# JiehongLin/SAM-6D

Measured on AMD Instinct MI355X. Metric: RGB-D frames/sec (SAM-6D per-frame hot path: SAM ViT-H encoder + ISM scoring + PEM), higher is better.
Workload: dtype bf16 (SAM ViT-H: 87 % of the step) + f16 (PEM ViT-B feature extractor) + f32 (ISM scoring, PEM point transformer and pose solvers); 1 GPU; LM-O single object: 32 frames/step/GPU, 640x480 RGB-D -> 1024^2 SAM input, P=128 proposals x 42 templates (scored in groups of 8 frames), 1 instance/frame, 2048 pts (PEM batch 32); sam_frames_per_launch_group=16, pem_vit_dtype=fp16 (set by bench.py; the library default is fp32)

## Files before the change

### sam6d_amd/csrc/s6d_attn_win16.h

```cpp
#pragma once
#include "s6d_attn_common.h"

namespace S6D_ATTN_NS {

#ifndef S6D_WIN16_STREAM
#define S6D_WIN16_STREAM 1
#endif
#ifndef S6D_WIN16_KSWZ
#define S6D_WIN16_KSWZ 1
#endif

template <int HD>
struct RelFrags {
  union { uint4 u; bf16x8 v; } rh[2][Cfg<HD>::KS], rw[2][Cfg<HD>::KS];
  __device__ __forceinline__ void load(const AttnParams &p, int lane) {
    using C = Cfg<HD>;
    const int g = lane >> 4, c = lane & 15;
#pragma unroll
    for (int jt = 0; jt < 2; ++jt)
#pragma unroll
      for (int ks = 0; ks < C::KS; ++ks) {
        rh[jt][ks].u = *reinterpret_cast<const uint4 *>(p.rel_h + (size_t)(jt * 16 + c) * C::HDP + ks * 32 + g * 8);
        rw[jt][ks].u = *reinterpret_cast<const uint4 *>(p.rel_w + (size_t)(jt * 16 + c) * C::HDP + ks * 32 + g * 8);
      }
  }
};

constexpr int W16_LT = 36;

template <int HD, int NR, int SRC>
__device__ __forceinline__ void win16_tables(const RelFrags<HD> &rf, int S, int qy0, int rstride,
                                             const bf16x8 (*qf)[Cfg<HD>::KS], float *tab, float (*twr)[4],
                                             float (*thv)[16], int lane) {
  using C = Cfg<HD>;
  const int g = lane >> 4, c = lane & 15;
#pragma unroll
  for (int n = 0; n < NR; ++n) {
    const int qy = min(qy0 + n * rstride, S - 1);
    f32x4 ah[2], aw[2];
#pragma unroll
    for (int jt = 0; jt < 2; ++jt) {
      ah[jt] = f32x4{0.f, 0.f, 0.f, 0.f};
      aw[jt] = f32x4{0.f, 0.f, 0.f, 0.f};
#pragma unroll
      for (int ks = 0; ks < C::KS; ++ks) {
        aw[jt] = S6D_ATTN_MFMA16(rf.rw[jt][ks].v, qf[n][ks], aw[jt]);
        ah[jt] = S6D_ATTN_MFMA16(rf.rh[jt][ks].v, qf[n][ks], ah[jt]);
      }
    }
#pragma unroll
    for (int jt = 0; jt < 2; ++jt)
      *reinterpret_cast<float4 *>(tab + c * W16_LT + jt * 16 + g * 4) =
          make_float4(aw[jt][0] * kLog2e, aw[jt][1] * kLog2e, aw[jt][2] * kLog2e, aw[jt][3] * kLog2e);
    S6D_WAVE_RENDEZVOUS();
#pragma unroll
    for (int r = 0; r < 4; ++r) {
      const int kx = g * 4 + r;
      const float v = tab[c * W16_LT + min(max(c - kx + S - 1, 0), 31)];
      twr[n][r] = (kx < S && c < S) ? v : -1e30f;
    }
    S6D_WAVE_RENDEZVOUS();
#pragma unroll
    for (int jt = 0; jt < 2; ++jt)
      *reinterpret_cast<float4 *>(tab + c * W16_LT + jt * 16 + g * 4) =
          make_float4(ah[jt][0] * kLog2e, ah[jt][1] * kLog2e, ah[jt][2] * kLog2e, ah[jt][3] * kLog2e);
    S6D_WAVE_RENDEZVOUS();
#pragma unroll
    for (int ky = 0; ky < SRC; ++ky) {
      const float v = tab[c * W16_LT + min(max(qy - ky + S - 1, 0), 31)];
      thv[n][ky] = ky < S ? v : -1e30f;
    }
    S6D_WAVE_RENDEZVOUS();
  }
}

struct Win16NoMid {
  __device__ __forceinline__ void operator()() const {}
};
template <int HD, int NS, int SRC, bool EXACT, int KROWT = Cfg<HD>::KROW, bool KSWZ = false, class MID = Win16NoMid>
__device__ __forceinline__ void win16_pass(const AttnParams &p, const u16 *Kl, const u16 *Vl, int S, int SR, int b,
                                           int wy, int wx, int head, int qy0, int rstride,
                                           const bf16x8 (&qf)[NS][Cfg<HD>::KS], const float (*twr)[4],
                                           const float (*thv)[16], int lane, MID mid = MID()) {
  using C = Cfg<HD>;
  const int g = lane >> 4, c = lane & 15;
  const int Cc = p.nh * HD;
  float sp[NS][SRC][4], m[NS];
#pragma unroll
  for (int n = 0; n < NS; ++n) m[n] = -1e29f;
  f32x4 cb[NS];
  {
    const float inv = 1.0f / p.scale_log2;
#pragma unroll
    for (int n = 0; n < NS; ++n)
#pragma unroll
      for (int r = 0; r < 4; ++r) cb[n][r] = twr[n][r] * inv;
  }
  bf16x8 kf[2][C::KS];
  const int gk = KSWZ ? (g ^ kswz(c)) : g;
  auto kload = [&](int ky, bf16x8 (&dst)[C::KS]) {
    const int kyc = EXACT ? ky : min(ky, SR - 1);
#pragma unroll
    for (int ks = 0; ks < C::KS; ++ks) {
      dst[ks] = *reinterpret_cast<const bf16x8 *>(Kl + (kyc * 16 + c) * KROWT + ks * 32 + gk * 8);
      if (KROWT < C::HDP && ks * 32 + 32 > HD && ks * 32 + g * 8 >= HD) {
        union { bf16x8 v; uint4 u; } z;
        z.u = make_uint4(0, 0, 0, 0);
        dst[ks] = z.v;
      }
    }
  };
  kload(0, kf[0]);
#pragma unroll
  for (int ky = 0; ky < SRC; ++ky) {
    if (ky + 1 < SRC) kload(ky + 1, kf[(ky + 1) & 1]);
    f32x4 acc[NS];
#pragma unroll
    for (int n = 0; n < NS; ++n) acc[n] = cb[n];
#pragma unroll
    for (int ks = 0; ks < C::KS; ++ks)
#pragma unroll
      for (int n = 0; n < NS; ++n)
        acc[n] = S6D_ATTN_MFMA16(kf[ky & 1][ks], qf[n][ks], acc[n]);
#pragma unroll
    for (int n = 0; n < NS; ++n) {
#pragma unroll
      for (int r = 0; r < 4; ++r) sp[n][ky][r] = acc[n][r];
      const float mk = __builtin_fmaf(fmaxf(fmaxf(acc[n][0], acc[n][1]), fmaxf(acc[n][2], acc[n][3])), p.scale_log2, thv[n][ky]);
      m[n] = fmaxf(m[n], mk);
    }
  }
#pragma unroll
  for (int n = 0; n < NS; ++n) {
    m[n] = fmaxf(m[n], __shfl_xor(m[n], 16));
    m[n] = fmaxf(m[n], __shfl_xor(m[n], 32));
  }
  f32x4 oacc[NS][C::DT], lacc[NS];
#pragma unroll
  for (int n = 0; n < NS; ++n) {
    lacc[n] = f32x4{0.f, 0.f, 0.f, 0.f};
#pragma unroll
    for (int dt = 0; dt < C::DT; ++dt) oacc[n][dt] = f32x4{0.f, 0.f, 0.f, 0.f};
  }
  union { bf16x8 v; u16 hh[8]; } ones;
#pragma unroll
  for (int i = 0; i < 8; ++i) ones.hh[i] = S6D_ATTN_ONE;
#pragma unroll
  for (int u = 0; u < SRC; u += 2) {
    if (u == ((SRC / 2 + 1) & ~1)) {
      __builtin_amdgcn_sched_barrier(0);
      mid();
      __builtin_amdgcn_sched_barrier(0);
    }
    if (EXACT || u < SR) {
      union { bf16x8 v; s16x4 q[2]; } va[C::DT];
      const u16 *vrow = Vl + (u * 16 + g * 4 + (c >> 2)) * C::VROW + (c & 3) * 4;
#pragma unroll
      for (int dt = 0; dt < C::DT; ++dt) {
        va[dt].q[0] = __builtin_amdgcn_ds_read_tr16_b64_v4i16((S6D_LDS(s16x4) *)(vrow + dt * 16));
        va[dt].q[1] = __builtin_amdgcn_ds_read_tr16_b64_v4i16((S6D_LDS(s16x4) *)(vrow + 16 * C::VROW + dt * 16));
      }
      union { bf16x8 v; u16 hh[8]; } pb[NS];
#pragma unroll
      for (int n = 0; n < NS; ++n)
#pragma unroll
        for (int h = 0; h < 2; ++h) {
          const float nb = thv[n][u + h] - m[n];
          for (int r = 0; r < 4; ++r) pb[n].hh[h * 4 + r] = f2bf(fast_exp2(__builtin_fmaf(sp[n][u + h][r], p.scale_log2, nb)));
        }
#pragma unroll
      for (int n = 0; n < NS; ++n) lacc[n] = S6D_ATTN_MFMA16(ones.v, pb[n].v, lacc[n]);
#pragma unroll
      for (int dt = 0; dt < C::DT; ++dt)
#pragma unroll
        for (int n = 0; n < NS; ++n)
          oacc[n][dt] = S6D_ATTN_MFMA16(va[dt].v, pb[n].v, oacc[n][dt]);
    }
  }
#pragma unroll
  for (int n = 0; n < NS; ++n) {
    const int qy = qy0 + n * rstride;
    const int y = wy * p.ws + qy, x = wx * p.ws + c;
    if ((qy < S) && c < S && (y < p.H) && (x < p.W)) {
      const float inv = 1.0f / lacc[n][0];
      u16 *dst = p.out + ((size_t)(b * p.H + y) * p.W + x) * (size_t)Cc + head * HD;
#pragma unroll
      for (int dt = 0; dt < C::DT; ++dt) {
        union { uint2 u2; u16 hh[4]; } o;
#pragma unroll
        for (int r = 0; r < 4; ++r) o.hh[r] = f2bf(oacc[n][dt][r] * inv);
        *reinterpret_cast<uint2 *>(dst + dt * 16 + g * 4) = o.u2;
      }
    }
  }
}

template <int HD, int SRC, int KROWT, bool KSWZ, class NEXTQ, class THISQ>
__device__ __forceinline__ void win16_pass_stream(const AttnParams &p, const u16 *Kl, const u16 *Vl, int S, int b, int wy, int wx,
                                                  int head, int qy0, int rstride, const bf16x8 (&qf)[2][Cfg<HD>::KS],
                                                  const float (*twr)[4], const float (*thv)[16], int lane, NEXTQ next_q, THISQ this_q) {
  using C = Cfg<HD>;
  constexpr int NS = 2;
  static_assert(SRC % 2 == 0 && SRC >= 4, "whole 32-key steps");
  const int g = lane >> 4, c = lane & 15;
  const int Cc = p.nh * HD;
  const int gk = KSWZ ? (g ^ kswz(c)) : g;
  f32x4 cb[NS];
  {
    const float inv = 1.0f / p.scale_log2;
#pragma unroll
    for (int n = 0; n < NS; ++n)
#pragma unroll
      for (int r = 0; r < 4; ++r) cb[n][r] = twr[n][r] * inv;
  }
  bf16x8 kf[2][C::KS];
  auto kload = [&](int ky, bf16x8 (&dst)[C::KS]) __attribute__((always_inline)) {
#pragma unroll
    for (int ks = 0; ks < C::KS; ++ks) {
      dst[ks] = *reinterpret_cast<const bf16x8 *>(Kl + (ky * 16 + c) * KROWT + ks * 32 + gk * 8);
      if (KROWT < C::HDP && ks * 32 + 32 > HD && ks * 32 + g * 8 >= HD) {
        union { bf16x8 v; uint4 u; } z;
        z.u = make_uint4(0, 0, 0, 0);
        dst[ks] = z.v;
      }
    }
  };
  auto scores = [&](const bf16x8 (&k)[C::KS], f32x4 (&acc)[NS]) __attribute__((always_inline)) {
#pragma unroll
    for (int n = 0; n < NS; ++n) acc[n] = cb[n];
#pragma unroll
    for (int ks = 0; ks < C::KS; ++ks)
#pragma unroll
      for (int n = 0; n < NS; ++n) acc[n] = S6D_ATTN_MFMA16(k[ks], qf[n][ks], acc[n]);
  };
  f32x4 s0[NS], s1[NS];
  kload(0, kf[0]);
  kload(1, kf[1]);
  scores(kf[0], s0);
  scores(kf[1], s1);
  float m[NS];
#pragma unroll
  for (int n = 0; n < NS; ++n) {
    const float m0 = __builtin_fmaf(fmaxf(fmaxf(s0[n][0], s0[n][1]), fmaxf(s0[n][2], s0[n][3])), p.scale_log2, thv[n][0]);
    const float m1 = __builtin_fmaf(fmaxf(fmaxf(s1[n][0], s1[n][1]), fmaxf(s1[n][2], s1[n][3])), p.scale_log2, thv[n][1]);
    float v = fmaxf(fmaxf(m0, m1), -1e29f);
    v = fmaxf(v, __shfl_xor(v, 16));
    v = fmaxf(v, __shfl_xor(v, 32));
    m[n] = v;
  }
  union { bf16x8 v; u16 hh[8]; } ones;
#pragma unroll
  for (int i = 0; i < 8; ++i) ones.hh[i] = S6D_ATTN_ONE;
  f32x4 oacc[NS][C::DT], lacc[NS];
  int round = 0;
  for (;;) {
#pragma unroll
    for (int n = 0; n < NS; ++n) {
      lacc[n] = f32x4{0.f, 0.f, 0.f, 0.f};
#pragma unroll
      for (int dt = 0; dt < C::DT; ++dt) oacc[n][dt] = f32x4{0.f, 0.f, 0.f, 0.f};
    }
#pragma unroll
    for (int u = 0; u < SRC; u += 2) {
      if (u > 0 || round > 0) {
        kload(u, kf[0]);
        kload(u + 1, kf[1]);
        scores(kf[0], s0);
        scores(kf[1], s1);
      }
      if (u == SRC - 2 && round == 0) {
        __builtin_amdgcn_sched_barrier(0);
        next_q();
        __builtin_amdgcn_sched_barrier(0);
      }
      union { bf16x8 v; s16x4 q[2]; } va[C::DT];
      const u16 *vrow = Vl + (u * 16 + g * 4 + (c >> 2)) * C::VROW + (c & 3) * 4;
#pragma unroll
      for (int dt = 0; dt < C::DT; ++dt) {
        va[dt].q[0] = __builtin_amdgcn_ds_read_tr16_b64_v4i16((S6D_LDS(s16x4) *)(vrow + dt * 16));
        va[dt].q[1] = __builtin_amdgcn_ds_read_tr16_b64_v4i16((S6D_LDS(s16x4) *)(vrow + 16 * C::VROW + dt * 16));
      }
      union { bf16x8 v; u16 hh[8]; } pb[NS];
#pragma unroll
      for (int n = 0; n < NS; ++n) {
        const float nb0 = thv[n][u] - m[n], nb1 = thv[n][u + 1] - m[n];
#pragma unroll
        for (int r = 0; r < 4; ++r) {
          pb[n].hh[r] = f2bf(fast_exp2(__builtin_fmaf(s0[n][r], p.scale_log2, nb0)));
          pb[n].hh[4 + r] = f2bf(fast_exp2(__builtin_fmaf(s1[n][r], p.scale_log2, nb1)));
        }
      }
#pragma unroll
      for (int n = 0; n < NS; ++n) lacc[n] = S6D_ATTN_MFMA16(ones.v, pb[n].v, lacc[n]);
#pragma unroll
      for (int dt = 0; dt < C::DT; ++dt)
#pragma unroll
        for (int n = 0; n < NS; ++n) oacc[n][dt] = S6D_ATTN_MFMA16(va[dt].v, pb[n].v, oacc[n][dt]);
    }
    bool any_bad = false;
#pragma unroll
    for (int n = 0; n < NS; ++n) {
      const int qy = qy0 + n * rstride;
      int ovf = 0;
#pragma unroll
      for (int dt = 0; dt < C::DT; ++dt)
#pragma unroll
        for (int r = 0; r < 4; ++r) ovf |= !(fabsf(oacc[n][dt][r]) < kNoMaxFinite);
      ovf |= __shfl_xor(ovf, 16);
      ovf |= __shfl_xor(ovf, 32);
      const bool bad = (qy < S) && (c < S) && (!(lacc[n][0] < kNoMaxSumLimit) || ovf);
      m[n] = bad ? m[n] + 96.0f : m[n];
      any_bad |= bad;
    }
    if (!__any(any_bad) || round >= 40) break;
    if (round == 0) this_q();
    ++round;
  }
  if (round > 0) next_q();
#pragma unroll
  for (int n = 0; n < NS; ++n) {
    const int qy = qy0 + n * rstride;
    const int y = wy * p.ws + qy, x = wx * p.ws + c;
    if ((qy < S) && c < S && (y < p.H) && (x < p.W)) {
      const float inv = 1.0f / lacc[n][0];
      u16 *dst = p.out + ((size_t)(b * p.H + y) * p.W + x) * (size_t)Cc + head * HD;
#pragma unroll
      for (int dt = 0; dt < C::DT; ++dt) {
        union { uint2 u2; u16 hh[4]; } o;
#pragma unroll
        for (int r = 0; r < 4; ++r) o.hh[r] = f2bf(oacc[n][dt][r] * inv);
        *reinterpret_cast<uint2 *>(dst + dt * 16 + g * 4) = o.u2;
      }
    }
  }
}

template <int HD, int WAVES>
__global__ __launch_bounds__(WAVES * 64) void attn_window16_kernel(AttnParams p) {
  using C = Cfg<HD>;
  S6D_ATTN_DYN_LDS(smem);
  const int S = p.S, SR = (S + 1) & ~1;
  u16 *Kl = reinterpret_cast<u16 *>(smem);
  u16 *Vl = Kl + (size_t)SR * 16 * C::KROW;
  float *tabs = reinterpret_cast<float *>(Vl + (size_t)SR * 16 * C::VROW);
  const int tid = threadIdx.x, wave = tid >> 6, lane = tid & 63;
  const int g = lane >> 4, c = lane & 15;
  float *tab = tabs + (size_t)wave * 16 * W16_LT;

  WinItem item;
  item.decode(p, blockIdx.x);
  const int head = item.head, wx = item.wx, wy = item.wy, b = item.b;
  const int Cc = p.nh * HD;
  constexpr int MAXROWS = 2;
  static_assert(2 * WAVES >= 16, "two rows per wave must cover 16 query rows");
  bf16x8 qfa[MAXROWS][C::KS];
#pragma unroll
  for (int i = 0; i < MAXROWS; ++i) {
    const int qy = wave + i * WAVES;
    const int y = wy * p.ws + qy, x = wx * p.ws + c;
    const bool qwin = c < S && qy < S, qimg = qwin && (y < p.H) && (x < p.W);
#pragma unroll
    for (int ks = 0; ks < C::KS; ++ks) {
      union { uint4 u; bf16x8 v; } t;
      const int d0 = ks * 32 + g * 8;
      const int dc = d0 < HD ? d0 : HD - 8;
      const size_t tokc = (size_t)(b * p.H + min(y, p.H - 1)) * p.W + min(x, p.W - 1);
      const u16 *src = qimg ? qkv_at(p, tokc, 0, head) + dc : p.qkv_bias + head * HD + dc;
      t.u = *reinterpret_cast<const uint4 *>(src);
      if (!(qwin && d0 < HD)) t.u = make_uint4(0, 0, 0, 0);
      qfa[i][ks] = t.v;
    }
  }
  RelFrags<HD> rf;
  rf.load(p, lane);
  constexpr int UN = 10;
  const int total = SR * 16 * (C::KPARTS + C::VPARTS);
  uint4 sv[UN];
  u16 *sdst[UN];
  auto issue = [&](int i0) {
#pragma unroll
    for (int n = 0; n < UN; ++n) {
      const int i = i0 + n * WAVES * 64;
      const int iq = min(i, total - 1);
      const bool isv = iq >= SR * 16 * C::KPARTS;
      const int ii = isv ? iq - SR * 16 * C::KPARTS : iq;
      const int parts = isv ? C::VPARTS : C::KPARTS;
      const int slot = ii / parts, part = ii - slot * parts;
      const int ky = slot >> 4, kx = slot & 15;
      const int y = wy * p.ws + ky, x = wx * p.ws + kx;
      sdst[n] = (i < total) ? (isv ? Vl + slot * C::VROW + part * 8 : Kl + slot * C::KROW + part * 8) : nullptr;
      const bool img = (y < p.H) && (x < p.W);
      const int dc = part * 8 < HD ? part * 8 : HD - 8;
      const size_t tokc = (size_t)(b * p.H + min(y, p.H - 1)) * p.W + min(x, p.W - 1);
      const int sel = (isv ? 2 : 1) * Cc + head * HD + dc;
      const u16 *src = img ? qkv_at(p, tokc, isv ? 2 : 1, head) + dc : p.qkv_bias + sel;
      sv[n] = *reinterpret_cast<const uint4 *>(src);
      if (!(ky < S && kx < S && part * 8 < HD)) sv[n] = make_uint4(0, 0, 0, 0);
    }
  };
  auto commit = [&]() {
#pragma unroll
    for (int n = 0; n < UN; ++n)
      if (sdst[n]) *reinterpret_cast<uint4 *>(sdst[n]) = sv[n];
  };
  const bool stage = !(kAbl & 1);
  if (stage) issue(tid);
  float twr[MAXROWS][4], thv[MAXROWS][16];
  if (!(kAbl & 2)) {
    if (S > WAVES) {
      if (S == 14)
        win16_tables<HD, 2, 14>(rf, S, wave, WAVES, qfa, tab, twr, thv, lane);
      else
        win16_tables<HD, 2, 16>(rf, S, wave, WAVES, qfa, tab, twr, thv, lane);
    } else if (wave < S) {
      win16_tables<HD, 1, 8>(rf, S, wave, WAVES, qfa, tab, twr, thv, lane);
    }
  }
  if (stage) {
    commit();
    for (int i0 = tid + UN * WAVES * 64; i0 < total; i0 += UN * WAVES * 64) {
      issue(i0);
      commit();
    }
  }
  __syncthreads();

  if (S <= WAVES) {
    if (wave < S && !(kAbl & 2)) {
      const bf16x8 (&q1)[1][C::KS] = reinterpret_cast<const bf16x8 (&)[1][C::KS]>(qfa[0]);
      win16_pass<HD, 1, 8, false>(p, Kl, Vl, S, SR, b, wy, wx, head, wave, WAVES, q1, twr, thv, lane);
    }
  } else if (!(kAbl & 2)) {
    static_assert(MAXROWS >= 2 || WAVES >= 16, "row bookkeeping");
    const bf16x8 (&q2)[2][C::KS] = reinterpret_cast<const bf16x8 (&)[2][C::KS]>(qfa[0]);
    if (S == 14) {
      win16_pass<HD, 2, 14, true>(p, Kl, Vl, S, SR, b, wy, wx, head, wave, WAVES, q2, twr, thv, lane);
    } else
      win16_pass<HD, 2, 16, false>(p, Kl, Vl, S, SR, b, wy, wx, head, wave, WAVES, q2, twr, thv, lane);
  }
}


template <int HD, bool S14>
__global__ __launch_bounds__(512) void attn_window16p_kernel(AttnParams p, int nitems) {
  using C = Cfg<HD>;
  constexpr int WAVES = 8;
  constexpr int KROWT = HD + 8, KCH = KROWT / 8, VCH = C::VROW / 8;
  S6D_ATTN_DYN_LDS(smem);
  const int S = p.S, SR = (S + 1) & ~1;
  const int kchunks = SR * 16 * KCH, vchunks = SR * 16 * VCH;
  const int kinstr = (kchunks + 63) >> 6, vinstr = (vchunks + 63) >> 6;
  const int kbytes = kinstr << 10, bufbytes = kbytes + (vinstr << 10);
  u16 *relh = reinterpret_cast<u16 *>(smem + 2 * bufbytes);
  u16 *relw = relh + 32 * C::HDP;
  const int tid = threadIdx.x, wave = __builtin_amdgcn_readfirstlane(tid >> 6), lane = tid & 63;
  const int g = lane >> 4, c = lane & 15;
  const int Cc = p.nh * HD;
  constexpr int RCH = C::HDP / 8;
  for (int i = tid; i < 2 * 32 * RCH; i += 512) {
    const bool w = i >= 32 * RCH;
    const int ii = w ? i - 32 * RCH : i;
    const int row = ii / RCH, ch = ii - row * RCH;
    reinterpret_cast<uint4 *>(w ? relw : relh)[row * RCH + (ch ^ ((row >> 2) & 3))] = reinterpret_cast<const uint4 *>(w ? p.rel_w : p.rel_h)[ii];
  }

  constexpr int MAXI = S14 ? 5 : 6;
  static_assert(((S14 ? 14 : 16) * 16 * (KCH > VCH ? KCH : VCH) + 63) / 64 <= WAVES * MAXI,
                "attn_window16p_kernel: K / V image has more DMA pieces than the unrolled slots (raise MAXI)");
  unsigned kvc[MAXI];
  {
#pragma unroll
    for (int i = 0; i < MAXI; ++i) {
      unsigned both = 0;
#pragma unroll
      for (int which = 1; which <= 2; ++which) {
        const int rowch = which == 1 ? KCH : VCH, nch = which == 1 ? kchunks : vchunks;
        const int k = wave + i * WAVES;
        const int j = min((k << 6) + lane, nch - 1);
        const int slot = j / rowch, pp = j - slot * rowch;
        const int ky = slot >> 4, kx = slot & 15;
        const int part = (S6D_WIN16_KSWZ && which == 1 && pp * 8 < HD) ? pp ^ kswz(kx) : pp;
        const bool inwin = ky < S && kx < S && part * 8 < HD;
        const unsigned v = (unsigned)(ky & 15) | ((unsigned)kx << 4) | ((unsigned)part << 8) | ((unsigned)inwin << 12);
        both |= which == 1 ? v : v << 16;
      }
      kvc[i] = both;
    }
  }
  auto stage_image = [&](const WinItem &it, int which, char *dst_base) __attribute__((always_inline)) {
    const int ninstr = which == 1 ? kinstr : vinstr;
    const int y0 = it.wy * p.ws, x0 = it.wx * p.ws, bH = it.b * p.H;
    const u16 *base = qkv_at(p, 0, which, it.head);
    const u16 *bias_base = p.qkv_bias + which * Cc + it.head * HD;
#pragma unroll
    for (int i = 0; i < MAXI; ++i) {
      const int k = wave + i * WAVES;
      if (k < ninstr) {
        unsigned cc = which == 1 ? kvc[i] : kvc[i] >> 16;
#ifndef HIPEMU
        asm volatile("" : "+v"(cc));
#endif
        const int ky = (int)(cc & 15u), kx = (int)((cc >> 4) & 15u), po = min((int)((cc >> 8) & 15u) * 8, HD - 8);
        const int y = y0 + ky, x = x0 + kx;
        const bool img = (y < p.H) && (x < p.W);
        const unsigned tok = (unsigned)(bH + min(y, p.H - 1)) * (unsigned)p.W + (unsigned)min(x, p.W - 1);
        const u16 *s_img = base + (size_t)tok * (size_t)p.tok_stride + po;
        const u16 *src = img ? s_img : bias_base + po;
        const void *sp = (cc >> 12) & 1u ? (const void *)src : (const void *)&g_attn_zero16;
        S6D_LDS(char) *dst = (S6D_LDS(char) *)dst_base + (k << 10);
        S6D_ATTN_DMA16(sp, dst);
      }
    }
  };
  constexpr int MAXROWS = 2;
  bf16x8 qfa[MAXROWS][C::KS];
  auto load_q = [&](const WinItem &it, bool raw, bf16x8 (&qdst)[MAXROWS][C::KS]) __attribute__((always_inline)) {
#pragma unroll
    for (int i = 0; i < MAXROWS; ++i) {
      const int qy = wave + i * WAVES;
      const int y = it.wy * p.ws + qy, x = it.wx * p.ws + c;
      const bool qwin = c < S && qy < S, qimg = qwin && (y < p.H) && (x < p.W);
#pragma unroll
      for (int ks = 0; ks < C::KS; ++ks) {
        union { uint4 u; bf16x8 v; } t;
        const int d0 = ks * 32 + g * 8;
        const int dc = d0 < HD ? d0 : HD - 8;
        const size_t tokc = (size_t)(it.b * p.H + min(y, p.H - 1)) * p.W + min(x, p.W - 1);
        const u16 *src = qimg ? qkv_at(p, tokc, 0, it.head) + dc : p.qkv_bias + it.head * HD + dc;
        t.u = *reinterpret_cast<const uint4 *>(src);
        if (!raw && !(qwin && d0 < HD)) t.u = make_uint4(0, 0, 0, 0);
        qdst[i][ks] = t.v;
      }
    }
  };
  auto mask_q = [&]() __attribute__((always_inline)) {
#pragma unroll
    for (int i = 0; i < MAXROWS; ++i) {
      const bool qwin = c < S && wave + i * WAVES < S;
#pragma unroll
      for (int ks = 0; ks < C::KS; ++ks) {
        union { uint4 u; bf16x8 v; } t;
        t.v = qfa[i][ks];
        if (!(qwin && ks * 32 + g * 8 < HD)) t.u = make_uint4(0, 0, 0, 0);
        qfa[i][ks] = t.v;
      }
    }
  };

  WinItem cur, nxt;
  int id = blockIdx.x;
  cur.decode(p, id);
  load_q(cur, false, qfa);
  stage_image(cur, 1, smem);
  stage_image(cur, 2, smem + kbytes);
  S6D_ATTN_VMCNT0();
  __syncthreads();
  int buf = 0;
  long long wtk[8] = {0, 0, 0, 0, 0, 0, 0, 0}, wsum[6] = {0, 0, 0, 0, 0, 0};
  for (; id < nitems; id += gridDim.x) {
    char *cb = smem + buf * bufbytes, *nb = smem + (buf ^ 1) * bufbytes;
    const bool more = id + (int)gridDim.x < nitems;
    S6D_TICK(wtk, 0);
    if (more) {
      nxt.decode(p, id + gridDim.x);
      stage_image(nxt, 1, nb);
    }
    float twr[MAXROWS][4], thv[MAXROWS][16];
    {
      RelFrags<HD> rf;
#pragma unroll
      for (int jt = 0; jt < 2; ++jt)
#pragma unroll
        for (int ks = 0; ks < C::KS; ++ks) {
          const int ro = (jt * 16 + c) * C::HDP + ((ks * 4 + g) ^ (((jt * 16 + c) >> 2) & 3)) * 8;
          rf.rh[jt][ks].u = *reinterpret_cast<const uint4 *>(relh + ro);
          rf.rw[jt][ks].u = *reinterpret_cast<const uint4 *>(relw + ro);
        }
      float *tab = reinterpret_cast<float *>(nb + kbytes) + (size_t)wave * 16 * W16_LT;
      if (S == 14)
        win16_tables<HD, 2, 14>(rf, S, wave, WAVES, qfa, tab, twr, thv, lane);
      else
        win16_tables<HD, 2, 16>(rf, S, wave, WAVES, qfa, tab, twr, thv, lane);
    }
    S6D_TICK(wtk, 1);
    __builtin_amdgcn_s_barrier();
    S6D_TICK(wtk, 2);
    if (more) stage_image(nxt, 2, nb + kbytes);
    S6D_TICK(wtk, 3);
    const u16 *Kl = reinterpret_cast<const u16 *>(cb), *Vl = reinterpret_cast<const u16 *>(cb + kbytes);
    const bf16x8 (&q2)[2][C::KS] = reinterpret_cast<const bf16x8 (&)[2][C::KS]>(qfa[0]);
    if (S14 && S6D_WIN16_STREAM) {
      auto next_q = [&]() __attribute__((always_inline)) {
        if (more) load_q(nxt, true, qfa);
      };
      auto this_q = [&]() __attribute__((always_inline)) { load_q(cur, false, qfa); };
      win16_pass_stream<HD, 14, KROWT, S6D_WIN16_KSWZ != 0>(p, Kl, Vl, S, cur.b, cur.wy, cur.wx, cur.head, wave, WAVES, q2, twr, thv, lane,
                                                            next_q, this_q);
    } else {
      auto mid = [&]() __attribute__((always_inline)) {
        if (more) load_q(nxt, true, qfa);
      };
      if (S14)
        win16_pass<HD, 2, 14, true, KROWT, S6D_WIN16_KSWZ != 0>(p, Kl, Vl, S, SR, cur.b, cur.wy, cur.wx, cur.head, wave, WAVES, q2, twr, thv, lane, mid);
      else
        win16_pass<HD, 2, 16, false, KROWT, S6D_WIN16_KSWZ != 0>(p, Kl, Vl, S, SR, cur.b, cur.wy, cur.wx, cur.head, wave, WAVES, q2, twr, thv, lane, mid);
    }
    S6D_TICK(wtk, 4);
    S6D_ATTN_VMCNT0();
    S6D_TICK(wtk, 5);
    __syncthreads();
    S6D_TICK(wtk, 6);
    if (S6D_G64_TIMING)
#pragma unroll
      for (int i = 0; i < 6; ++i) wsum[i] += wtk[i + 1] - wtk[i];
    mask_q();
    cur = nxt;
    buf ^= 1;
  }
  if (S6D_G64_TIMING && blockIdx.x == 8 && lane == 0) {
    long long *dbg = reinterpret_cast<long long *>(p.out + (size_t)p.B * p.H * p.W * p.nh * HD);
#pragma unroll
    for (int i = 0; i < 6; ++i) dbg[wave * 6 + i] = wsum[i];
  }
}

template <int HD>
static int launch_win16(AttnParams p, hipStream_t st) {
  using C = Cfg<HD>;
  constexpr int WAVES = 8;
  const int SR = (p.S + 1) & ~1;
  if (p.S > WAVES) {
    const int kin = (SR * 16 * (HD + 8) / 8 + 63) / 64, vin = (SR * 16 * C::VROW / 8 + 63) / 64;
    const size_t lds = (size_t)2 * (kin + vin) * 1024 + (size_t)2 * 32 * C::HDP * 2;
    const int nitems = p.B * p.nwy * p.nwx * p.nh;
    if (lds <= 160 * 1024 && (size_t)WAVES * 16 * W16_LT * 4 <= (size_t)vin * 1024) {
      int grid = nitems < 256 ? nitems : 256;
      if (s6d::g_s6d_persistent_grid_limit > 0 && s6d::g_s6d_persistent_grid_limit < grid) grid = s6d::g_s6d_persistent_grid_limit;
      if (grid >= 8) grid &= ~7;
      if (p.S == 14) {
        launch_lds(attn_window16p_kernel<HD, true>, grid, 512, lds, st, p, nitems);
      } else {
        launch_lds(attn_window16p_kernel<HD, false>, grid, 512, lds, st, p, nitems);
      }
      return launch_status();
    }
  }
  const size_t lds = (size_t)SR * 16 * (C::KROW + C::VROW) * 2 + (size_t)WAVES * 16 * W16_LT * 4;
  if (lds > 160 * 1024) return S6D_EUNSUPPORTED;
  launch_lds(attn_window16_kernel<HD, WAVES>, (unsigned)(p.B * p.nwy * p.nwx * p.nh), WAVES * 64, lds, st, p);
  return launch_status();
}

}
```

Baseline: 165.3 frames/s.

## Map only valid query rows to waves in streamed window-16 attention

In the persistent window-16 attention kernel's streaming path, query rows are now assigned to waves from the window's valid extent. Edge windows clipped by the image border get fewer rows per wave, and narrow windows pack two half-rows of 8 columns into one 16-lane strip. Waves with no valid rows skip the relative-position table and attention pass entirely, and waves with one row run a single-row variant. This targets wasted MFMA and exp work on padded rows in partial windows, at the cost of more index arithmetic, extra template instantiations and possible wave imbalance.

```diff
diff --git a/sam6d_amd/csrc/s6d_attn_win16.h b/sam6d_amd/csrc/s6d_attn_win16.h
--- a/sam6d_amd/csrc/s6d_attn_win16.h
+++ b/sam6d_amd/csrc/s6d_attn_win16.h
@@ -68,6 +68,53 @@
 #pragma unroll
     for (int ky = 0; ky < SRC; ++ky) {
       const float v = tab[c * W16_LT + min(max(qy - ky + S - 1, 0), 31)];
+      thv[n][ky] = ky < S ? v : -1e30f;
+    }
+    S6D_WAVE_RENDEZVOUS();
+  }
+}
+
+template <int HD, int NR, int SRC, class QAT>
+__device__ __forceinline__ void win16_tables_at(const RelFrags<HD> &rf, int S, const bf16x8 (*qf)[Cfg<HD>::KS], float *tab,
+                                                float (*twr)[4], float (*thv)[16], int lane, QAT qat) {
+  using C = Cfg<HD>;
+  const int g = lane >> 4, c = lane & 15;
+#pragma unroll
+  for (int n = 0; n < NR; ++n) {
+    int qy, qx;
+    const bool qok = qat(n, qy, qx);
+    f32x4 ah[2], aw[2];
+#pragma unroll
+    for (int jt = 0; jt < 2; ++jt) {
+      ah[jt] = f32x4{0.f, 0.f, 0.f, 0.f};
+      aw[jt] = f32x4{0.f, 0.f, 0.f, 0.f};
+#pragma unroll
+      for (int ks = 0; ks < C::KS; ++ks) {
+        aw[jt] = S6D_ATTN_MFMA16(rf.rw[jt][ks].v, qf[n][ks], aw[jt]);
+        ah[jt] = S6D_ATTN_MFMA16(rf.rh[jt][ks].v, qf[n][ks], ah[jt]);
+      }
+    }
+#pragma unroll
+    for (int jt = 0; jt < 2; ++jt)
+      *reinterpret_cast<float4 *>(tab + c * W16_LT + jt * 16 + g * 4) =
+          make_float4(aw[jt][0] * kLog2e, aw[jt][1] * kLog2e, aw[jt][2] * kLog2e, aw[jt][3] * kLog2e);
+    S6D_WAVE_RENDEZVOUS();
+#pragma unroll
+    for (int r = 0; r < 4; ++r) {
+      const int kx = g * 4 + r;
+      const float v = tab[c * W16_LT + min(max(qx - kx + S - 1, 0), 31)];
+      twr[n][r] = (kx < S && qok) ? v : -1e30f;
+    }
+    S6D_WAVE_RENDEZVOUS();
+#pragma unroll
+    for (int jt = 0; jt < 2; ++jt)
+      *reinterpret_cast<float4 *>(tab + c * W16_LT + jt * 16 + g * 4) =
+          make_float4(ah[jt][0] * kLog2e, ah[jt][1] * kLog2e, ah[jt][2] * kLog2e, ah[jt][3] * kLog2e);
+    S6D_WAVE_RENDEZVOUS();
+    const float *trow = tab + c * W16_LT + ((qok ? qy : 0) + S - SRC);
+#pragma unroll
+    for (int ky = 0; ky < SRC; ++ky) {
+      const float v = trow[SRC - 1 - ky];
       thv[n][ky] = ky < S ? v : -1e30f;
     }
     S6D_WAVE_RENDEZVOUS();
@@ -195,12 +242,11 @@
   }
 }
 
-template <int HD, int SRC, int KROWT, bool KSWZ, class NEXTQ, class THISQ>
-__device__ __forceinline__ void win16_pass_stream(const AttnParams &p, const u16 *Kl, const u16 *Vl, int S, int b, int wy, int wx,
-                                                  int head, int qy0, int rstride, const bf16x8 (&qf)[2][Cfg<HD>::KS],
-                                                  const float (*twr)[4], const float (*thv)[16], int lane, NEXTQ next_q, THISQ this_q) {
+template <int HD, int NS, int SRC, int KROWT, bool KSWZ, class QAT, class NEXTQ, class THISQ>
+__device__ __forceinline__ void win16_pass_stream(const AttnParams &p, const u16 *Kl, const u16 *Vl, int b, int head,
+                                                  const bf16x8 (&qf)[NS][Cfg<HD>::KS], const float (*twr)[4], const float (*thv)[16],
+                                                  int lane, QAT qat, NEXTQ next_q, THISQ this_q) {
   using C = Cfg<HD>;
-  constexpr int NS = 2;
   static_assert(SRC % 2 == 0 && SRC >= 4, "whole 32-key steps");
   const int g = lane >> 4, c = lane & 15;
   const int Cc = p.nh * HD;
@@ -300,7 +346,8 @@
     bool any_bad = false;
 #pragma unroll
     for (int n = 0; n < NS; ++n) {
-      const int qy = qy0 + n * rstride;
+      int y, x;
+      const bool qok = qat(n, y, x);
       int ovf = 0;
 #pragma unroll
       for (int dt = 0; dt < C::DT; ++dt)
@@ -308,7 +355,7 @@
         for (int r = 0; r < 4; ++r) ovf |= !(fabsf(oacc[n][dt][r]) < kNoMaxFinite);
       ovf |= __shfl_xor(ovf, 16);
       ovf |= __shfl_xor(ovf, 32);
-      const bool bad = (qy < S) && (c < S) && (!(lacc[n][0] < kNoMaxSumLimit) || ovf);
+      const bool bad = qok && (!(lacc[n][0] < kNoMaxSumLimit) || ovf);
       m[n] = bad ? m[n] + 96.0f : m[n];
       any_bad |= bad;
     }
@@ -319,9 +366,8 @@
   if (round > 0) next_q();
 #pragma unroll
   for (int n = 0; n < NS; ++n) {
-    const int qy = qy0 + n * rstride;
-    const int y = wy * p.ws + qy, x = wx * p.ws + c;
-    if ((qy < S) && c < S && (y < p.H) && (x < p.W)) {
+    int y, x;
+    if (qat(n, y, x)) {
       const float inv = 1.0f / lacc[n][0];
       u16 *dst = p.out + ((size_t)(b * p.H + y) * p.W + x) * (size_t)Cc + head * HD;
 #pragma unroll
@@ -439,6 +485,31 @@
       win16_pass<HD, 2, 16, false>(p, Kl, Vl, S, SR, b, wy, wx, head, wave, WAVES, q2, twr, thv, lane);
   }
 }
+
+struct Win16Strips {
+  int y0, x0, vr, vc, wave, waves, ns;
+  int two;
+  __device__ __forceinline__ void set(const AttnParams &p, const WinItem &it, int wave_, int waves_) {
+    wave = wave_;
+    waves = waves_;
+    y0 = it.wy * p.ws;
+    x0 = it.wx * p.ws;
+    vr = min(p.S, p.H - y0);
+    vc = min(p.S, p.W - x0);
+    two = vc <= 8;
+    const int strips = two ? (vr + 1) >> 1 : vr;
+    ns = (wave < strips) + (wave + waves < strips);
+  }
+  __device__ __forceinline__ bool query(int i, int c, int &qy, int &qx) const {
+    const int s = wave + i * waves;
+#ifndef HIPEMU
+    asm volatile("" : "+v"(c));
+#endif
+    qy = two ? 2 * s + (c >> 3) : s;
+    qx = two ? (c & 7) : c;
+    return i < ns && qy < vr && qx < vc;
+  }
+};
 
 
 template <int HD, bool S14>
@@ -546,11 +617,60 @@
       }
     }
   };
+  auto load_q_at = [&](const WinItem &it, const Win16Strips &mp, bool raw, bf16x8 (&qdst)[MAXROWS][C::KS]) __attribute__((always_inline)) {
+#pragma unroll
+    for (int i = 0; i < MAXROWS; ++i)
+      if (i < mp.ns) {
+        int qy, qx;
+        const bool ok = mp.query(i, c, qy, qx);
+        const int y = mp.y0 + qy, x = mp.x0 + qx;
+#pragma unroll
+        for (int ks = 0; ks < C::KS; ++ks) {
+          union { uint4 u; bf16x8 v; } t;
+          const int d0 = ks * 32 + g * 8;
+          const int dc = d0 < HD ? d0 : HD - 8;
+          const size_t tokc = (size_t)(it.b * p.H + min(y, p.H - 1)) * p.W + min(x, p.W - 1);
+          const u16 *src = ok ? qkv_at(p, tokc, 0, it.head) + dc : p.qkv_bias + it.head * HD + dc;
+          t.u = *reinterpret_cast<const uint4 *>(src);
+          if (!raw && !(ok && d0 < HD)) t.u = make_uint4(0, 0, 0, 0);
+          qdst[i][ks] = t.v;
+        }
+      }
+  };
+  auto mask_q_at = [&](const Win16Strips &mp) __attribute__((always_inline)) {
+#pragma unroll
+    for (int i = 0; i < MAXROWS; ++i) {
+      int qy, qx;
+      const bool ok = mp.query(i, c, qy, qx);
+#pragma unroll
+      for (int ks = 0; ks < C::KS; ++ks) {
+        union { uint4 u; bf16x8 v; } t;
+        t.v = qfa[i][ks];
+        if (!(ok && ks * 32 + g * 8 < HD)) t.u = make_uint4(0, 0, 0, 0);
+        qfa[i][ks] = t.v;
+      }
+    }
+  };
+  constexpr bool STREAM = S14 && S6D_WIN16_STREAM;
 
   WinItem cur, nxt;
   int id = blockIdx.x;
   cur.decode(p, id);
-  load_q(cur, false, qfa);
+  Win16Strips mc, mn;
+  mc.set(p, cur, wave, WAVES);
+  if (STREAM) {
+#pragma unroll
+    for (int i = 0; i < MAXROWS; ++i)
+#pragma unroll
+      for (int ks = 0; ks < C::KS; ++ks) {
+        union { uint4 u; bf16x8 v; } z;
+        z.u = make_uint4(0, 0, 0, 0);
+        qfa[i][ks] = z.v;
+      }
+    load_q_at(cur, mc, false, qfa);
+  } else {
+    load_q(cur, false, qfa);
+  }
   stage_image(cur, 1, smem);
   stage_image(cur, 2, smem + kbytes);
   S6D_ATTN_VMCNT0();
@@ -561,12 +681,14 @@
     char *cb = smem + buf * bufbytes, *nb = smem + (buf ^ 1) * bufbytes;
     const bool more = id + (int)gridDim.x < nitems;
     S6D_TICK(wtk, 0);
+    mn = mc;
     if (more) {
       nxt.decode(p, id + gridDim.x);
+      if (STREAM) mn.set(p, nxt, wave, WAVES);
       stage_image(nxt, 1, nb);
     }
     float twr[MAXROWS][4], thv[MAXROWS][16];
-    {
+    if (!STREAM || mc.ns > 0) {
       RelFrags<HD> rf;
 #pragma unroll
       for (int jt = 0; jt < 2; ++jt)
@@ -577,7 +699,12 @@
           rf.rw[jt][ks].u = *reinterpret_cast<const uint4 *>(relw + ro);
         }
       float *tab = reinterpret_cast<float *>(nb + kbytes) + (size_t)wave * 16 * W16_LT;
-      if (S == 14)
+      auto qat = [&](int n, int &qy, int &qx) __attribute__((always_inline)) { return mc.query(n, c, qy, qx); };
+      if (STREAM && mc.ns == 2)
+        win16_tables_at<HD, 2, 14>(rf, S, qfa, tab, twr, thv, lane, qat);
+      else if (STREAM)
+        win16_tables_at<HD, 1, 14>(rf, S, qfa, tab, twr, thv, lane, qat);
+      else if (S == 14)
         win16_tables<HD, 2, 14>(rf, S, wave, WAVES, qfa, tab, twr, thv, lane);
       else
         win16_tables<HD, 2, 16>(rf, S, wave, WAVES, qfa, tab, twr, thv, lane);
@@ -589,13 +716,26 @@
     S6D_TICK(wtk, 3);
     const u16 *Kl = reinterpret_cast<const u16 *>(cb), *Vl = reinterpret_cast<const u16 *>(cb + kbytes);
     const bf16x8 (&q2)[2][C::KS] = reinterpret_cast<const bf16x8 (&)[2][C::KS]>(qfa[0]);
-    if (S14 && S6D_WIN16_STREAM) {
+    if (STREAM) {
       auto next_q = [&]() __attribute__((always_inline)) {
-        if (more) load_q(nxt, true, qfa);
+        if (more) load_q_at(nxt, mn, true, qfa);
       };
-      auto this_q = [&]() __attribute__((always_inline)) { load_q(cur, false, qfa); };
-      win16_pass_stream<HD, 14, KROWT, S6D_WIN16_KSWZ != 0>(p, Kl, Vl, S, cur.b, cur.wy, cur.wx, cur.head, wave, WAVES, q2, twr, thv, lane,
-                                                            next_q, this_q);
+      auto this_q = [&]() __attribute__((always_inline)) { load_q_at(cur, mc, false, qfa); };
+      auto qat = [&](int n, int &y, int &x) __attribute__((always_inline)) {
+        int qy, qx;
+        const bool ok = mc.query(n, c, qy, qx);
+        y = mc.y0 + qy;
+        x = mc.x0 + qx;
+        return ok;
+      };
+      if (mc.ns == 2) {
+        win16_pass_stream<HD, 2, 14, KROWT, S6D_WIN16_KSWZ != 0>(p, Kl, Vl, cur.b, cur.head, q2, twr, thv, lane, qat, next_q, this_q);
+      } else if (mc.ns == 1) {
+        const bf16x8 (&q1)[1][C::KS] = reinterpret_cast<const bf16x8 (&)[1][C::KS]>(qfa[0]);
+        win16_pass_stream<HD, 1, 14, KROWT, S6D_WIN16_KSWZ != 0>(p, Kl, Vl, cur.b, cur.head, q1, twr, thv, lane, qat, next_q, this_q);
+      } else {
+        next_q();
+      }
     } else {
       auto mid = [&]() __attribute__((always_inline)) {
         if (more) load_q(nxt, true, qfa);
@@ -613,7 +753,12 @@
     if (S6D_G64_TIMING)
 #pragma unroll
       for (int i = 0; i < 6; ++i) wsum[i] += wtk[i + 1] - wtk[i];
-    mask_q();
+    if (STREAM) {
+      mask_q_at(mn);
+      mc = mn;
+    } else {
+      mask_q();
+    }
     cur = nxt;
     buf ^= 1;
   }
```

Result: no change. 166.0 frames/s (median of 6 runs) (+0.4%).
